# jennalandy/bayesNMF

Measured on AMD Instinct MI355X. Metric: Gibbs iters/sec at K=96, G=10k, N=20; per-chain scaling at 1/2/4/8 GPUs, higher is better.
Workload: dtype f64; 1 GPU; Poisson-Gamma fixed rank N=20, K=96 x G=10000 synthetic counts, one chain per GPU, stats mode, record_sample into a 1000-deep device ring (on) and a metrics row every iteration; chains=1, seed=1, sum_M=40006177, record_window=1000

## Files before the change

bayesnmf_amd/csrc/api.hip:

```cpp
#include <hip/hip_runtime.h>
#include <hip/hip_ext.h>
#include <chrono>
#include <climits>
#include <cmath>
#include <cstdarg>
#include <cstdio>
#include <cstdlib>
#include <cstring>
#include <cerrno>
#include <algorithm>
#include <map>
#include <atomic>
#include <condition_variable>
#include <mutex>
#include <string>
#include <thread>
#include <vector>
#include <fcntl.h>
#include <sys/file.h>
#include <sys/stat.h>
#include <unistd.h>
#include "kernels.h"
#include "zalloc_reg.h"
#include "zalloc_sort.h"
// ... 47 lines not shown
  DevPool& P = g_pool[dev];
  {
    std::lock_guard<std::mutex> lk(P.m);
    auto it = P.free_blocks.find(bytes);
    if (it != P.free_blocks.end()) { *out = it->second; P.free_blocks.erase(it); P.cached -= bytes; P.live[*out] = bytes; return hipSuccess; }
  }
  hipError_t e = hipMalloc(out, bytes);
  if (e != hipSuccess) { (void)hipGetLastError(); pool_drop(dev); e = hipMalloc(out, bytes); }
  if (e == hipSuccess) { std::lock_guard<std::mutex> lk(P.m); P.live[*out] = bytes; }
  return e;
}
template <class T> static hipError_t dmalloc(T** out, size_t bytes) { return dmalloc_raw((void**)out, bytes); }
static hipError_t dfree(void* p) {
  if (!p) return hipSuccess;
  int dev = -1;
  if (hipGetDevice(&dev) != hipSuccess || dev < 0 || dev >= 64) return hipFree(p);
  DevPool& P = g_pool[dev];
  {
    std::lock_guard<std::mutex> lk(P.m);
    auto it = P.live.find(p);
    if (it != P.live.end()) {
      const size_t bytes = it->second;
      P.live.erase(it);
      if (P.cached + bytes <= pool_cap()) { P.free_blocks.insert({bytes, p}); P.cached += bytes; return hipSuccess; }
    }
  }
  return hipFree(p);
}


#include "zplan.h"

struct Arr { double* d = nullptr; size_t n = 0; int stride = 1; bool set = false; std::vector<int> redraw; double* ring = nullptr;
             bool slab = false; };

struct Pipe {
  bool side_valid = false, side_main = false, flags_valid = false, side_ev_stale = false;
  int gate_f0 = 1;
  uint32_t z_gate_next = 0, z_gated_for = 0;
  bool red_pending = false, red_issued = false, red_on_side2 = false; uint32_t red_t = 0; int red_row = 0;
  uint32_t ct_pending = 0, mh_etail_pending = 0;
  bool mh_prep_valid = false, mh_pipe_valid = false;
  int z_expanded_iter = 0;
  void invalidate_prepared() { side_valid = false; side_main = false; mh_prep_valid = false; mh_pipe_valid = false; }
};

enum class ZKind { none , general , reg , tile, step, sort };

struct ZTile : ZTilePlan { double* dMhat = nullptr; };
struct ZSort {
  bool pk = false, shared = false;
  ZSGeom g{}; int nblk = 0, w = 0; size_t lds = 0;
  int it16 = 0, qmax = ZS_QMAX;
  int nempty = 0;
  uint32_t* dItems = nullptr; ZSBlock* dBlocks = nullptr; int* dCols = nullptr; int32_t* dM = nullptr; unsigned long long* dProf = nullptr;
  double* dMh = nullptr;
  uint32_t *dRec = nullptr, *dRecRing = nullptr; size_t recwords = 0; bool eager = false;
  int x_cols = 0; size_t x_lds = 0;
};
struct ZStep {
  ZPGeom g{}; int ns = 0 , gbp = 0; size_t lds = 0; bool it16 = false;
  uint32_t* dItems = nullptr; ZPWg* dWgs = nullptr; ZPBatch* dBatches = nullptr; ZPStep* dSteps = nullptr; int* dCols = nullptr;
};
struct Rank : RankPlan { double *dCol = nullptr, *dMhat = nullptr; uint32_t* dSync = nullptr; void* dDbg = nullptr; };
struct Mh : MhPlan {
  bool side_tail = true;
  bool side_main = true;
  bool no_reg = false;
  bool e_k128 = false;
  int e_gw = 0;
  double *dMhat = nullptr, *dAccPn = nullptr, *dAccEpart = nullptr, *dEt = nullptr; int* dNzE = nullptr;
  int32_t* dMt = nullptr; double* dMtf = nullptr;
};

struct Scratch { unsigned char* p = nullptr; size_t bytes = 0; };

struct bnmf_handle {
  bnmf_config cfg{};
  int device = 0;
  hipStream_t stream = nullptr;
  hipStream_t side = nullptr;
  hipStream_t side2 = nullptr;
  hipEvent_t ev_draw = nullptr, ev_side = nullptr, ev_sideP = nullptr, ev_p = nullptr, ev_z = nullptr, ev_red = nullptr, ev_rank = nullptr;
  std::vector<void*> owned;
  int gate_forced = -1;
  int draw_bw = 0;
  double* dScal = nullptr;
  unsigned* dDrawOwn = nullptr; unsigned draw_seq = 0;
  int dbg_draw_no_p = 0;
  int dbg_main_delay_us = 0;
  int dbg_allside_delay_us = 0;
  int dbg_side_delay_us = 0;
  double* E_alt = nullptr;
  const void* z_attr_kernel = nullptr;
  Pipe pipe;
  int iter = 0;
  bool inited = false;
  Dev dev{};
  Arr arr[BNMF_ID_MAX];
  int32_t *dM = nullptr, *dZsumK = nullptr, *dZsumG = nullptr, *dZ = nullptr;
  double* dMf = nullptr;
  int* dR = nullptr; int* dRedraw = nullptr;
  std::vector<int32_t> fixedP;
  int n_fixed = 0; int* dFixedP = nullptr;
  double *dEsum = nullptr, *dPsum = nullptr, *dlpPn = nullptr, *dlpE = nullptr, *dcol = nullptr;
  double* hMetrics = nullptr;
// ... 189 lines not shown
  if (int rc = check_args("bnmf_create", cfg, M, out)) return rc;
  return create_handle(cfg, M, nullptr, out);
}

int bnmf_create_f64(const bnmf_config* cfg, const double* M, bnmf_handle** out) {
  if (int rc = check_args("bnmf_create_f64", cfg, M, out)) return rc;
  const size_t K = cfg->K, G = cfg->G;
  if (cfg->likelihood == BNMF_NORMAL) {
    for (size_t g = 0; g < G; ++g)
      for (size_t k = 0; k < K; ++k)
        if (!std::isfinite(M[k + K * g])) return fail(BNMF_EINVAL, "bnmf_create_f64: M[%zu, %zu] = %g is not finite", k, g, M[k + K * g]);
    return create_handle(cfg, nullptr, M, out);
  }
  if (cfg->likelihood != BNMF_POISSON) return fail(BNMF_EMODEL, "likelihood must be one of normal, poisson");
  std::vector<int32_t> mi(K * G);
  for (size_t g = 0; g < G; ++g)
    for (size_t k = 0; k < K; ++k) {
      const double v = M[k + K * g];
      if (!(v >= 0.0 && v <= 2147483647.0 && v == std::floor(v)))
        return fail(BNMF_EINVAL, "bnmf_create_f64: non-integer count M[%zu, %zu] = %g (likelihood = poisson takes whole numbers in [0, 2^31 - 1])", k, g, v);
      mi[k + K * g] = (int32_t)v;
    }
  return bnmf_create(cfg, mi.data(), out);
}

static int build_zsort(bnmf_handle* h, const int32_t* M, bool reg_ok, const Switches& sw) {
  const bnmf_config& c = h->cfg;
  const size_t K = c.K, G = c.G, N = c.N;
  ZSort& z = h->zs;
  ZSortPlan p;
  if (int rc = plan_zsort(M, K, G, N, c.save_Z != 0, h->maxM, reg_ok, h->n_cu, sw, p)) return rc;
  if (!p.ok) return 0;
  if (p.it16) HIPCHK(hupload(h, &z.dItems, p.items16.data(), p.items16.size() * sizeof(uint16_t), (p.items16.size() * sizeof(uint16_t) + 3) & ~(size_t)3));
  else HIPCHK(hupload(h, &z.dItems, p.items.data(), p.items.size() * sizeof(uint32_t)));
  z.it16 = p.it16 ? 1 : 0; z.qmax = p.qmax;
  HIPCHK(hupload(h, &z.dBlocks, p.blocks.data(), p.blocks.size() * sizeof(ZSBlock)));
  HIPCHK(hupload(h, &z.dCols, p.cols.data(), p.cols.size() * sizeof(int)));
  HIPCHK(hupload(h, &z.dM, p.Mblk.data(), p.Mblk.size() * sizeof(int32_t)));
  HIPCHK(hzeroed(h, &z.dMh, 3 * K * G * sizeof(double)));
  if (c.save_Z) {
    const size_t hw = (N + 1) / 2;
    z.recwords = p.items.size() * hw;
    HIPCHK(hmalloc(h, &z.dRec, z.recwords * sizeof(uint32_t)));
    z.eager = sw.z_eager;
    const size_t lds_max = 160 * 1024;
    z.x_cols = std::max(1, std::min(p.GBc, zexpand_cols((int)K, (int)N, lds_max)));
    z.x_lds = ((size_t)z.x_cols * N * ((K + 1) / 2) * 4 + 15) & ~(size_t)15;
    if (z.x_lds > lds_max) return fail(BNMF_EINVAL, "bnmf_create: K = %zu, N = %zu: a column of Z does not fit the LDS of k_zexpand", K, N);
    HIPCHK(hipFuncSetAttribute((const void*)k_zexpand, hipFuncAttributeMaxDynamicSharedMemorySize, 160 * 1024));
  }
  z.g = ZSGeom{p.KP, p.GBc, p.nb};
  z.shared = p.shared;
  z.nblk = p.nblk; z.w = p.W; z.pk = p.pk; z.nempty = p.nempty;
  z.lds = (zsort_shared_bytes((int)K, (int)N, p.KP, p.GBc, p.pk) + (size_t)p.W * zsort_wave_bytes(p.nblk, (int)N) + 15) & ~(size_t)15;
  h->zkind = ZKind::sort;
#ifdef ZSPROF
  HIPCHK(hzeroed(h, &z.dProf, (8 + 3 * 16 * 8) * sizeof(unsigned long long)));
#endif
  return 0;
}

static int build_zstep(bnmf_handle* h, const int32_t* M, const Switches& sw) {
  const bnmf_config& c = h->cfg;
  ZStep& z = h->zp;
  ZStepPlan p;
  if (int rc = plan_zstep(M, c.K, c.G, c.N, c.save_Z != 0, h->n_cu, sw, p)) return rc;
  if (!p.ok) return 0;
  z.it16 = p.it16;
  if (p.it16) HIPCHK(hupload(h, &z.dItems, p.items16.data(), p.items16.size() * sizeof(uint16_t), (p.items16.size() * sizeof(uint16_t) + 3) & ~(size_t)3));
  else HIPCHK(hupload(h, &z.dItems, p.items.data(), p.items.size() * sizeof(uint32_t)));
  HIPCHK(hupload(h, &z.dWgs, p.wgs.data(), p.wgs.size() * sizeof(ZPWg)));
  HIPCHK(hupload(h, &z.dBatches, p.batches.data(), p.batches.size() * sizeof(ZPBatch)));
  HIPCHK(hupload(h, &z.dSteps, p.steps.data(), p.steps.size() * sizeof(ZPStep)));
  HIPCHK(hupload(h, &z.dCols, p.cols.data(), p.cols.size() * sizeof(int)));
  z.g = ZPGeom{p.nch, p.nwg, nullptr};
#ifdef ZPPROF
  HIPCHK(hzeroed(h, &z.g.prof, 8 * sizeof(unsigned long long)));
#endif
  z.ns = p.W; z.gbp = p.GBP;
  z.lds = (zstep_shared_bytes((int)c.N, p.GBP) + p.W * zstep_wave_bytes(p.L) + 15) & ~(size_t)15;
  h->zkind = ZKind::step;
  return 0;
}

static std::mutex g_stream_mtx;
static std::vector<hipStream_t> g_stream_pool[64];
static int take_stream(int device, hipStream_t* out, int kind = 0) {
  (void)kind;
  if (device < 0 || device >= 64) return fail(BNMF_EINVAL, "device ordinal %d out of range", device);
  {
    std::lock_guard<std::mutex> lock(g_stream_mtx);
    auto& v = g_stream_pool[device];
    if (!v.empty()) { *out = v.back(); v.pop_back(); return 0; }
  }
  HIPCHK(hipStreamCreateWithFlags(out, hipStreamNonBlocking));
  return 0;
}
static void give_stream(int device, hipStream_t st, int kind = 0) {
  (void)kind;
  if (!st) return;
  if (device < 0 || device >= 64) { hipStreamDestroy(st); return; }
  std::lock_guard<std::mutex> lock(g_stream_mtx);
  g_stream_pool[device].push_back(st);
}
struct CachedBuf { void* p; size_t bytes; };
static std::mutex g_ring_mtx;
// ... 1017 lines not shown
```

bayesnmf_amd/csrc/sweep.h:

```cpp
#include <cassert>

static int need_hyper(bnmf_handle* h, std::initializer_list<int> ids) {
  for (int id : ids) if (!h->arr[id].d) return fail(BNMF_EUNSET, "hyper-prior array id %d was not set (fill_hyperprior_params, R/setup.R:15-88)", id);
  return 0;
}
static int ensure_metrics(bnmf_handle* h, size_t rows) {
  if (rows <= h->metrics_rows) return 0;
  HIPCHK(hipStreamSynchronize(h->stream));
  HIPCHK(hipHostFree(h->hMetrics));
  h->hMetrics = nullptr; h->dMetrics = nullptr;
  h->metrics_rows = rows;
  HIPCHK(hipHostMalloc((void**)&h->hMetrics, rows * BNMF_NMETRIC * sizeof(double), hipHostMallocMapped));
  HIPCHK(hipHostGetDevicePointer((void**)&h->dMetrics, h->hMetrics, 0));
  HIPCHK(hfree(h, h->dRaw));
  HIPCHK(hmalloc(h, &h->dRaw, rows * 8 * sizeof(double)));
  refresh_dev(h);
  return 0;
}
static void set_slot(const bnmf_handle* h, Dev& d, uint32_t t) {
  const size_t sl = t % 3u, G = h->cfg.G, N = h->cfg.N;
  d.colsse = h->dcol + sl * 3 * G; d.colll = d.colsse + G; d.colkl = d.colsse + 2 * G;
  d.lpE_part = h->dlpE + sl * (size_t)h->nblkE;
  d.lpPn = h->dlpPn + sl * N;
}
// ... 204 lines not shown
}
template <bool SZ, int ZT_, bool LEAN_>
static int launch_ztile(bnmf_handle* h, uint32_t t) {
  auto kern = k_zalloc_tile<SZ, ZT_, LEAN_>;
  if (int rc = raise_lds_limit(h, (const void*)kern)) return rc;
  const ZArgs za = zargs(h);
  hipLaunchKernelGGL(kern, dim3(h->zt.grid), dim3(ZT_), h->zt.lds, h->stream, za, h->zt.dMhat, t, h->zt.g);
  hipLaunchKernelGGL(k_colmetrics<256>, dim3((h->cfg.G + 3) / 4), dim3(256), 0, h->stream, za, (const double*)h->zt.dMhat);
  if (h->zt.g.dbg) {
    unsigned long long v[8];
    hipStreamSynchronize(h->stream);
    hipMemcpy(v, h->zt.g.dbg, sizeof v, hipMemcpyDeviceToHost);
    hipMemset(h->zt.g.dbg, 0, sizeof v);
    if (v[0]) fprintf(stderr, "[ztile t=%u] waves %llu grid %d w %d lds %zu  per wave: phase1 %.1f  phase2 %.1f  flush %.1f  columns %.1f  kernel %.1f (s_memtime ticks)\n",
                      t, v[0], h->zt.grid, h->zt.w, h->zt.lds, (double)v[1] / v[0], (double)v[2] / v[0], (double)v[3] / v[0], (double)v[4] / v[0], (double)v[5] / v[0]);
  }
  return 0;
}
template <bool SZ, int ZT_>
static int launch_zalloc_t(bnmf_handle* h, uint32_t t) {
  if (h->zkind == ZKind::tile) return (h->zt.lean && ZT_ == 1024) ? launch_ztile<SZ, ZT_, (ZT_ == 1024)>(h, t) : launch_ztile<SZ, ZT_, false>(h, t);
  if (h->zkind == ZKind::general) return launch_z(h, t, k_zalloc<SZ, ZT_>, h->dev, ZT_);
#ifdef BNMF_DIAG
  if (h->z_ablate) return launch_zreg_t<SZ, ZT_, true>(h, t);
#endif
  return launch_zreg_t<SZ, ZT_, false>(h, t);
}
static int zs_prio() { static const int v = getenv("BNMF_ZSPRIO") ? atoi(getenv("BNMF_ZSPRIO")) : 1; return v; }
static uint32_t* zs_rec_at(const bnmf_handle* h, uint32_t t) {
  if (!h->zs.dRec) return nullptr;
  return h->zs.dRecRing ? h->zs.dRecRing + (size_t)((t - 1) % (uint32_t)h->wcap) * h->zs.recwords : h->zs.dRec;
}
static void launch_zexpand(bnmf_handle* h, uint32_t t) {
  const ZSArgs sa{zargs(h), h->zs.dItems, h->zs.dBlocks, h->zs.dCols, h->zs.dM, h->zs.it16, h->zs.qmax, zs_rec_at(h, t), nullptr, 0, 0, h->zs.dProf};
  hipLaunchKernelGGL(k_zexpand, dim3(h->zs.g.nblocks), dim3(ZX_T), h->zs.x_lds, h->stream, sa, h->zs.x_cols);
  h->pipe.z_expanded_iter = (int)t;
}
static int ensure_Z(bnmf_handle* h) {
  if (h->zkind != ZKind::sort || !h->zs.dRec || !h->cfg.save_Z || h->iter < 1 || h->pipe.z_expanded_iter == h->iter) return 0;
  HIPCHK(hipSetDevice(h->device));
  launch_zexpand(h, (uint32_t)h->iter);
  HIPCHK(hipGetLastError());
  HIPCHK(hipStreamSynchronize(h->stream));
  return 0;
}
template <int ZT_>
static int launch_zsort_t(bnmf_handle* h, uint32_t t) {
  const ZSArgs sa{zargs(h), h->zs.dItems, h->zs.dBlocks, h->zs.dCols, h->zs.dM, h->zs.it16, h->zs.qmax, zs_rec_at(h, t), h->zs.dMh + (size_t)(t % 3u) * h->cfg.K * h->cfg.G, zs_prio(), h->zs.shared ? 1 : 0, h->zs.dProf};
  auto go = [&](auto kern) -> int {
    if (int rc = raise_lds_limit(h, (const void*)kern)) return rc;
    hipLaunchKernelGGL(kern, dim3(h->zs.g.nblocks), dim3(ZT_), h->zs.lds, h->stream, sa, t, h->zs.g);
    return 0;
  };
#ifdef BNMF_FASTBUILD
  if (h->zs.nblk != 4) return fail(BNMF_EMODEL, "BNMF_FASTBUILD: only N = 16..20");
  return h->zs.pk ? go(k_zalloc_sort<ZT_, 4, true>) : go(k_zalloc_sort<ZT_, 4, false>);
#else
  if (h->zs.pk) switch (h->zs.nblk) {
    case 1: return go(k_zalloc_sort<ZT_, 1, true>);
    case 2: return go(k_zalloc_sort<ZT_, 2, true>);
    case 3: return go(k_zalloc_sort<ZT_, 3, true>);
    case 4: return go(k_zalloc_sort<ZT_, 4, true>);
    default: return go(k_zalloc_sort<ZT_, 5, true>);
  }
  switch (h->zs.nblk) {
    case 1: return go(k_zalloc_sort<ZT_, 1, false>);
    case 2: return go(k_zalloc_sort<ZT_, 2, false>);
    case 3: return go(k_zalloc_sort<ZT_, 3, false>);
    case 4: return go(k_zalloc_sort<ZT_, 4, false>);
    default: return go(k_zalloc_sort<ZT_, 5, false>);
  }
#endif
}
static int launch_zsort(bnmf_handle* h, uint32_t t) {
#ifdef BNMF_FASTBUILD
  if (h->zs.w == 14) return launch_zsort_t<896>(h, t);
  if (h->zs.w != 12) return fail(BNMF_EMODEL, "BNMF_FASTBUILD: only 12 or 14 waves");
  return launch_zsort_t<768>(h, t);
#else
  switch (h->zs.w) {
    case 16: return launch_zsort_t<1024>(h, t);
    case 14: return launch_zsort_t<896>(h, t);
    case 12: return launch_zsort_t<768>(h, t);
    case 8: return launch_zsort_t<512>(h, t);
    case 6: return launch_zsort_t<384>(h, t);
    default: return launch_zsort_t<256>(h, t);
  }
#endif
}
static int launch_zstep(bnmf_handle* h, uint32_t t) {
  const ZPArgs pa{zargs(h), h->zp.dItems, h->zp.it16 ? 1 : 0, h->zp.dWgs, h->zp.dBatches, h->zp.dSteps, h->zp.dCols};
  auto go = [&](auto kern) -> int {
    if (int rc = raise_lds_limit(h, (const void*)kern)) return rc;
    hipLaunchKernelGGL(kern, dim3(h->zp.g.nwg), dim3(h->zp.ns * 64), h->zp.lds, h->stream, pa, t, h->zp.g);
    return 0;
  };
  return h->zp.gbp == 40 ? go(k_zalloc_step<4, 40, 8>) : go(k_zalloc_step<4, 32, 8>);
}
static int launch_zalloc(bnmf_handle* h, uint32_t t) {
  int w = 0;
  switch (h->zkind) {
    case ZKind::none: return fail(BNMF_ESTATE, "launch_zalloc: the handle allocates no counts");
    case ZKind::sort:
      if (int rc = launch_zsort(h, t)) return rc;
      if (h->cfg.save_Z && h->zs.eager) launch_zexpand(h, t);
      return 0;
// ... 466 lines not shown
```

bayesnmf_amd/csrc/zalloc_sort.h:

```cpp
#pragma once

namespace bnmf {

constexpr int ZS_QMAX = 32;
constexpr int ZS_QMAX16 = 64;
constexpr int ZS_NMAX = 25;

struct ZSBlock { int item0, ntask, col0, ncols; };
struct ZSGeom { int KP, GBc, nblocks; };
struct ZSArgs {
  ZArgs a;
  const uint32_t* items;
  const ZSBlock* blocks;
  const int* cols;
  const int32_t* Mblk;
  int it16, qmax;
  uint32_t* rec;
  double* mh;
  int prio;
  int shared;
  unsigned long long* prof;
};
#ifdef ZSPROF
#define ZSTIC(i) const uint64_t zstic_##i = __builtin_amdgcn_s_memtime()
#define ZSTOC(i) zsprof[i] += __builtin_amdgcn_s_memtime() - zstic_##i
#define ZSSTAMP(j) do { if (s.prof && zs_sel >= 0 && lane == 0) s.prof[8 + (zs_sel * 16 + wave) * 8 + (j)] = __builtin_amdgcn_s_memrealtime(); } while (0)
#else
#define ZSTIC(i)
#define ZSTOC(i)
#define ZSSTAMP(j)
#endif
#define BNMF_HD __host__ __device__ inline
BNMF_HD int zsort_zrows(int N, bool pk) { return pk ? (N + 1) / 2 : N; }
BNMF_HD size_t zsort_shared_bytes(int K, int N, int KP, int GBc, bool pk) {
  size_t w = (size_t)zsort_zrows(N, pk) * (KP + GBc) + GBc + 4;
  w = (w + 3) & ~(size_t)3;
  return (w * 4 + ((size_t)K * N + (size_t)N * GBc) * 8 + 15) & ~(size_t)15;
}
BNMF_HD size_t zsort_wave_bytes(int NBLK, int N) { return (size_t)NBLK * 64 * 16 + (size_t)(2 * ((N + 1) / 2)) * 64 * 4; }

template <int ZT, int NBLK , bool PK>
__global__ __launch_bounds__(ZT) __attribute__((amdgpu_waves_per_eu(4))) void k_zalloc_sort(ZSArgs s, uint32_t t, ZSGeom zg) {
  constexpr int NPV = NBLK - 1;
  constexpr int NC = 5 * NBLK;
  constexpr int NMIN = NBLK == 1 ? 1 : 5 * (NBLK - 1) + 1;
  extern __shared__ __attribute__((aligned(16))) unsigned char smem[];
  const ZArgs& d = s.a;
  const int tid = threadIdx.x, lane = tid & 63, wave = tid >> 6;
  const int K = d.K, N = d.N, KP = zg.KP, GBc = zg.GBc;
  const int HW = (N + 1) >> 1;
  const int ZR = PK ? HW : N;
  const ZSBlock bk = s.blocks[blockIdx.x];
  uint32_t* zG = (uint32_t*)smem;
  uint32_t* zK = zG + (size_t)ZR * KP;
  int* colid = (int*)(zK + (size_t)ZR * GBc);
  uint32_t* ticket = (uint32_t*)(colid + GBc);
  const size_t w32 = (((size_t)ZR * (KP + GBc) + GBc + 4) + 3) & ~(size_t)3;
  const int32_t* Mb = s.Mblk + (size_t)K * bk.col0;
  double* Pl = (double*)(smem + w32 * 4);
  double* ae = Pl + (size_t)K * N;
  unsigned char* wbase = smem + zsort_shared_bytes(K, N, KP, GBc, PK) + (size_t)wave * zsort_wave_bytes(NBLK, N);
  u4* tblk = (u4*)wbase;
  uint32_t* hist = (uint32_t*)(tblk + NBLK * 64);
#ifdef ZSPROF
  uint64_t zsprof[8] = {0, 0, 0, 0, 0, 0, 0, 1};
#endif
#ifdef ZSPROF
  int zs_ntask = 0;
  const int zs_sel = blockIdx.x == 0 ? 0 : blockIdx.x == 128 ? 1 : blockIdx.x == gridDim.x - 1 ? 2 : -1;
#endif
  ZSSTAMP(0);
  ZSTIC(6);
  ZSTIC(0);
  for (int i = lane; i < 2 * HW * 64; i += 64) hist[i] = 0;
  {
    constexpr int UA = 2, UP = 4;
    const int nP = K * N, nA = N * bk.ncols;
    const int nchunk = max(max((nA + UA * ZT - 1) / (UA * ZT), (nP + UP * ZT - 1) / (UP * ZT)), 1);
    for (int ch = 0; ch < nchunk; ++ch) {
      int gcol[UA], an_i[UA], ax[UA];
      double an[UA], pv[UP], ev[UA];
#pragma unroll
      for (int u = 0; u < UA; ++u) {
        const int i = (ch * UA + u) * ZT + tid;
        const bool ok = i < nA;
        const int gl = ok ? i / N : 0, n = ok ? i - gl * N : 0;
        ax[u] = ok ? n * GBc + gl : -1; an_i[u] = n;
        gcol[u] = s.cols[bk.col0 + gl];
        an[u] = d.A[n];
      }
#pragma unroll
      for (int u = 0; u < UP; ++u) { const int i = (ch * UP + u) * ZT + tid; pv[u] = i < nP ? d.P[i] : 0.0; }
#pragma unroll
      for (int u = 0; u < UA; ++u) ev[u] = d.E[an_i[u] + (size_t)N * gcol[u]];
#pragma unroll
      for (int u = 0; u < UP; ++u) { const int i = (ch * UP + u) * ZT + tid; if (i < nP) Pl[i] = pv[u]; }
#pragma unroll
      for (int u = 0; u < UA; ++u) if (ax[u] >= 0) ae[ax[u]] = an[u] * ev[u];
    }
    for (int i = tid; i < bk.ncols; i += ZT) colid[i] = s.cols[bk.col0 + i];
    for (int i = tid; i < ZR * KP; i += ZT) zG[i] = 0;
    for (int i = tid; i < ZR * GBc; i += ZT) zK[i] = 0;
    if (tid == 0) *ticket = 0;
  }
  ZSSTAMP(1);
  __syncthreads();
  ZSTOC(0);
  ZSSTAMP(2);
  if (s.prio) __builtin_amdgcn_s_setprio(2);
  const int nthr = N - 1;
  const int ntot = bk.ntask;
  const uint32_t hlb = lds_off(hist + lane);
  auto next_task = [&]() -> int {
    int tk = 0;
    if (lane == 0) tk = (int)__hip_atomic_fetch_add(ticket, 1u, __ATOMIC_RELAXED, __HIP_MEMORY_SCOPE_WORKGROUP);
    return __builtin_amdgcn_readlane(tk, 0);
  };
  for (int task = next_task(); task < ntot; task = next_task()) {
    {
    ZSTIC(1);
    uint32_t it;
    if (s.it16) {
      const uint32_t r = ((const uint16_t*)s.items)[(size_t)bk.item0 + (size_t)task * 64 + lane];
      it = r == 0xFFFFu ? 0xFFFFFFFFu : ((r & 127u) | (((r >> 7) & 63u) << 10) | ((r >> 13) << 16));
    } else it = s.items[(size_t)bk.item0 + (size_t)task * 64 + lane];
    const bool valid = it != 0xFFFFFFFFu;
    const int k = valid ? (int)(it & 1023u) : 0, gl = valid ? (int)((it >> 10) & 63u) : 0;
    const int q0 = valid ? (int)(it >> 16) * s.qmax : 0;
    const int m = Mb[k + (size_t)K * gl];
    const int g = colid[gl];
    int nq = 0, npad = 0;
    bool any = false;
    uint32_t pv[NPV > 0 ? NPV : 1];
    {
      const double* Pk = Pl + k;
      const double* ag = ae + gl;
      double cs[NC];
      double c = 0.0;
#pragma unroll
      for (int n = 0; n < NC; ++n) { if (n < NMIN || n < N) c = c + Pk[(size_t)K * n] * ag[(size_t)n * GBc]; cs[n] = c; }
      if (valid && c > 0.0 && m > 0) {
        const int qt = (m + 3) >> 2;
        nq = min(s.qmax, qt - q0);
        npad = (q0 + nq == qt) ? ((4 - (m & 3)) & 3) : 0;
      }
      if (valid && q0 == 0) s.mh[(size_t)k + (size_t)K * (size_t)g] = c;
      any = __builtin_amdgcn_ballot_w64(nq > 0) != 0;
      if (any) {
      const double scale = 4294967296.0 / c;
#pragma unroll
      for (int j = 0; j < NBLK; ++j) {
        uint32_t tv[5];
#pragma unroll
        for (int i = 0; i < 5; ++i) {
          const int n = 5 * j + i;
          tv[i] = 0xFFFFFFFFu;
          if (n < NC - 1 && (n < NMIN - 1 || n < nthr)) tv[i] = cvt_u32_sat(cs[n] * scale);
        }
        tblk[j * 64 + lane] = u4{tv[0], tv[1], tv[2], tv[3]};
        if (j < NPV) pv[j] = tv[4];
      }
      }
    }
    const uint32_t celem = (uint32_t)k + (uint32_t)K * (uint32_t)g;
    auto quad = [&](int qidx, uint32_t inc0, uint32_t inc1, uint32_t inc2, uint32_t inc3) {
      const u32x4 w = philox4x32_7((uint32_t)qidx, celem, t, BNMF_V_Z, d.k0, d.k1);
      const uint32_t u0 = min(w.x, 0xFFFFFFFEu), u1 = min(w.y, 0xFFFFFFFEu), u2 = min(w.z, 0xFFFFFFFEu), u3 = min(w.w, 0xFFFFFFFEu);
      uint32_t j0 = 0, j1 = 0, j2 = 0, j3 = 0;
#pragma unroll
      for (int p = 0; p < NPV; ++p) cmp_acc4(pv[p], u0, u1, u2, u3, j0, j1, j2, j3);
      const u4 k0 = tblk[j0 * 64 + lane], k1 = tblk[j1 * 64 + lane], k2 = tblk[j2 * 64 + lane], k3 = tblk[j3 * 64 + lane];
      const uint32_t b0 = 5 * j0 + (k0.x <= u0) + (k0.y <= u0) + (k0.z <= u0) + (k0.w <= u0);
      const uint32_t b1 = 5 * j1 + (k1.x <= u1) + (k1.y <= u1) + (k1.z <= u1) + (k1.w <= u1);
      const uint32_t b2 = 5 * j2 + (k2.x <= u2) + (k2.y <= u2) + (k2.z <= u2) + (k2.w <= u2);
      const uint32_t b3 = 5 * j3 + (k3.x <= u3) + (k3.y <= u3) + (k3.z <= u3) + (k3.w <= u3);
      lds_add(mad24(b0, 256, hlb), inc0);
      lds_add(mad24(b1, 256, hlb), inc1);
      lds_add(mad24(b2, 256, hlb), inc2);
      lds_add(mad24(b3, 256, hlb), inc3);
    };
    wave_lds_fence();
    ZSTOC(1);
#ifdef ZSPROF
    if (zs_ntask == 0) ZSSTAMP(6);
#endif
    ZSTIC(2);
    if (any) for (int i = 0; __builtin_amdgcn_ballot_w64(i < nq - 1) != 0; ++i)
      if (i < nq - 1) quad(q0 + i, 1u, 1u, 1u, 1u);
    if (nq > 0) quad(q0 + nq - 1, 1u, npad > 2 ? 0u : 1u, npad > 1 ? 0u : 1u, npad > 0 ? 0u : 1u);
    wave_lds_fence();
    ZSTOC(2);
#ifdef ZSPROF
    if (zs_ntask == 0) ZSSTAMP(7);
    ++zs_ntask;
#endif
    ZSTIC(3);
    if (s.rec) {
      uint32_t* rt = s.rec + ((size_t)(bk.item0 >> 6) + (size_t)task) * (size_t)HW * 64 + lane;
      for (int w = 0; w < HW; ++w) rt[(size_t)w * 64] = hist[(2 * w) * 64 + lane] | (hist[(2 * w + 1) * 64 + lane] << 16);
    }
    if (nq > 0) {
      const uint32_t zgb = lds_off(zG) + ((uint32_t)k << 2), zkb = lds_off(zK) + ((uint32_t)gl << 2);
      for (int w = 0; w < HW; ++w) {
        const uint32_t v0 = hist[(2 * w) * 64 + lane], v1 = hist[(2 * w + 1) * 64 + lane];
        const uint32_t v = v0 | (v1 << 16);
        if (v) {
          hist[(2 * w) * 64 + lane] = 0; hist[(2 * w + 1) * 64 + lane] = 0;
          if (PK) {
            lds_add(zgb + (uint32_t)w * (uint32_t)KP * 4u, v); lds_add(zkb + (uint32_t)w * (uint32_t)GBc * 4u, v);
          } else {
            const uint32_t lo = v & 0xFFFFu, hi = v >> 16;
            if (lo) { lds_add(zgb + (uint32_t)(2 * w) * (uint32_t)KP * 4u, lo); lds_add(zkb + (uint32_t)(2 * w) * (uint32_t)GBc * 4u, lo); }
            if (hi) { lds_add(zgb + (uint32_t)(2 * w + 1) * (uint32_t)KP * 4u, hi); lds_add(zkb + (uint32_t)(2 * w + 1) * (uint32_t)GBc * 4u, hi); }
          }
        }
      }
    }
    wave_lds_fence();
    ZSTOC(3);
    }
  }
  ZSSTAMP(3);
  ZSTIC(5);
  __syncthreads();
  ZSTOC(5);
  ZSSTAMP(4);
  {
  ZSTIC(0);
  for (int i = tid; i < N * bk.ncols; i += ZT) {
    const int gl = i / N, n = i - gl * N;
    const uint32_t v = PK ? (zK[(size_t)(n >> 1) * GBc + gl] >> ((n & 1) << 4)) & 0xFFFFu : zK[(size_t)n * GBc + gl];
    if (s.shared) { if (v) atomicAdd(&d.ZsumK[n + (size_t)N * colid[gl]], (int32_t)v); }
    else d.ZsumK[n + (size_t)N * colid[gl]] = (int32_t)v;
  }
  for (int i = tid; i < K * N; i += ZT) {
    const int kk = i % K, n = i / K;
    const uint32_t v = PK ? (zG[(size_t)(n >> 1) * KP + kk] >> ((n & 1) << 4)) & 0xFFFFu : zG[(size_t)n * KP + kk];
    if (v) atomicAdd(&d.ZsumG[kk + (size_t)K * n], (int32_t)v);
  }
  ZSTOC(0);
  }
  ZSTOC(6);
  ZSSTAMP(5);
#ifdef ZSPROF
  if (s.prof && lane == 0) for (int i = 0; i < 8; ++i) atomicAdd(&s.prof[i], (unsigned long long)zsprof[i]);
#endif
  if (d.gate0 && blockIdx.x == 0 && tid == 0) {
    unsigned spins = 0;
    while (__hip_atomic_load(d.gate0, __ATOMIC_RELAXED, __HIP_MEMORY_SCOPE_AGENT) < d.gate_epoch ||
           __hip_atomic_load(d.gate1, __ATOMIC_RELAXED, __HIP_MEMORY_SCOPE_AGENT) < d.gate_epoch) {
      __builtin_amdgcn_s_sleep(2);
      if (++spins > (1u << 24)) { __hip_atomic_store(d.gate_err, 2, __ATOMIC_RELAXED, __HIP_MEMORY_SCOPE_AGENT); break; }
    }
  }
}

constexpr int ZX_T = 1024;
BNMF_HD int zexpand_cols(int K, int N, size_t lds_bytes) { return (int)(lds_bytes / ((size_t)N * (size_t)((K + 1) / 2) * 4)); }
__global__ __launch_bounds__(ZX_T) void k_zexpand(ZSArgs s, int cols_per_pass) {
  extern __shared__ __attribute__((aligned(16))) unsigned char smem[];
  uint32_t* slab = (uint32_t*)smem;
  const ZArgs& d = s.a;
  const int tid = threadIdx.x, K = d.K, N = d.N, KH = (K + 1) >> 1, HW = (N + 1) >> 1;
  const ZSBlock bk = s.blocks[blockIdx.x];
  const int nslots = bk.ntask * 64;
  for (int c0 = 0; c0 < bk.ncols; c0 += cols_per_pass) {
    const int nc = min(cols_per_pass, bk.ncols - c0);
    for (int i = tid; i < nc * N * KH; i += ZX_T) slab[i] = 0u;
    __syncthreads();
    for (int i = tid; i < nslots; i += ZX_T) {
      uint32_t it;
      if (s.it16) { const uint32_t r = ((const uint16_t*)s.items)[(size_t)bk.item0 + i]; it = r == 0xFFFFu ? 0xFFFFFFFFu : ((r & 127u) | (((r >> 7) & 63u) << 10)); }
      else it = s.items[(size_t)bk.item0 + i];
      if (it == 0xFFFFFFFFu) continue;
      const int k = (int)(it & 1023u), gl = (int)((it >> 10) & 63u) - c0;
      if (gl < 0 || gl >= nc) continue;
      const uint32_t* rt = s.rec + ((size_t)((bk.item0 + i) >> 6)) * (size_t)HW * 64 + (i & 63);
      uint32_t* sc = slab + (size_t)gl * N * KH + (k >> 1);
      const int sh = (k & 1) << 4;
      for (int w = 0; w < HW; ++w) {
        const uint32_t v = rt[(size_t)w * 64];
        if (v & 0xFFFFu) atomicAdd(sc + (size_t)(2 * w) * KH, (v & 0xFFFFu) << sh);
        if (v >> 16) atomicAdd(sc + (size_t)(2 * w + 1) * KH, (v >> 16) << sh);
      }
    }
// ... 23 lines not shown
```

bayesnmf_amd/csrc/zplan.h:

```cpp

static const int ENV_UNSET = INT_MIN;
static bool env_set(const char* name) { return getenv(name) != nullptr; }
static int env_int(const char* name, int unset = ENV_UNSET, int lo = INT_MIN, int hi = INT_MAX) {
  const char* e = getenv(name);
  return e ? std::max(lo, std::min(hi, atoi(e))) : unset;
}
static bool env_flag(const char* name, bool unset) { const char* e = getenv(name); return e ? atoi(e) != 0 : unset; }
static double env_real(const char* name, double unset) { const char* e = getenv(name); return e ? atof(e) : unset; }
struct Switches {
  bool devlock = true;
  int gate = -1, serial = -1;
  bool mh_side_main = true, mh_side_tail = true;
  bool draw_no_p = false;
  int main_delay_us = 0, allside_delay_us = 0, side_delay_us = 0;
  bool rank_dbg = false, zt_dbg = false;
  bool z_eager = false;
  int ablate = 0;
  bool rank_half = true; long rank_grid = 0;
  bool mhe_k128 = false, mh_pipe = true; int mhe_gw = 0;
  bool z_reg = true, z_chunk = false, z_tile = true, z_nolean = false;
  int zw = ENV_UNSET, z_grid = ENV_UNSET;
  bool zsort = true, zs_spread = true, zs_it16 = true, zs_pk = true;
  int zs_lds_kb = ENV_UNSET, zs_w = ENV_UNSET, zs_qmax = 0;
  bool zstep = true, zp_it16 = true; int zp_gb = 0;
  static Switches from_env() {
    Switches s;
    s.devlock = env_flag("BNMF_DEVLOCK", true);
    s.gate = env_set("BNMF_GATE") ? (int)env_flag("BNMF_GATE", false) : -1;
    s.serial = env_set("BNMF_SERIAL") ? (int)env_flag("BNMF_SERIAL", false) : -1;
    s.mh_side_main = env_flag("BNMF_MHSIDE", true); s.mh_side_tail = env_flag("BNMF_MHSIDETAIL", true);
    s.draw_no_p = env_flag("BNMF_DEBUG_DRAW_NO_P", false);
    s.main_delay_us = env_int("BNMF_DEBUG_MAIN_DELAY_US", 0, 0, 20000);
    s.allside_delay_us = env_int("BNMF_DEBUG_ALLSIDE_DELAY_US", 0, 0, 20000);
    s.side_delay_us = env_int("BNMF_DEBUG_SIDE_DELAY_US", 0, 0, 20000);
    s.rank_dbg = env_set("BNMF_RANKDBG"); s.zt_dbg = env_set("BNMF_ZTDBG");
    s.z_eager = env_flag("BNMF_ZEAGER", false);
#ifdef BNMF_DIAG
    s.ablate = env_int("BNMF_ABLATE", 0);
#endif
    s.rank_half = env_flag("BNMF_RANKHALF", true);
    if (const char* e = getenv("BNMF_RANKGRID")) s.rank_grid = atol(e);
    s.mhe_k128 = env_flag("BNMF_MHE_K128", false); s.mh_pipe = env_flag("BNMF_MHPIPE", true);
    { const int v = env_int("BNMF_MHE_GW", 0); s.mhe_gw = v == 32 ? 32 : v == 16 ? 16 : 0; }
    s.z_reg = env_flag("BNMF_ZREG", true); s.z_chunk = env_flag("BNMF_ZCHUNK", false);
    s.z_tile = env_flag("BNMF_ZTILE", true); s.z_nolean = env_set("BNMF_ZNOLEAN");
    s.zw = env_int("BNMF_ZW"); s.z_grid = env_int("BNMF_ZGRID");
    s.zsort = env_flag("BNMF_ZSORT", true); s.zs_spread = env_flag("BNMF_ZSSPREAD", true);
    s.zs_it16 = env_flag("BNMF_ZSIT16", true); s.zs_pk = env_flag("BNMF_ZSPK", true);
    s.zs_lds_kb = env_int("BNMF_ZSLDS"); s.zs_w = env_int("BNMF_ZSW"); s.zs_qmax = env_int("BNMF_ZSQMAX", 0);
    s.zstep = env_flag("BNMF_ZSTEP", true); s.zp_it16 = env_flag("BNMF_ZPIT16", true); s.zp_gb = env_int("BNMF_ZPGB", 0);
    return s;
  }
};

struct RankPlan { bool reg = false, half = false; int grid = 0; };
static RankPlan plan_rank(size_t K, size_t G, int n_cu, int occ_reg, int occ_gen, const Switches& sw) {
  RankPlan p;
  const long NB = ((long)G + RK_MAXC - 1) / RK_MAXC;
  const long wg_needed = (NB + RK_CW - 1) / RK_CW;
  auto cap = [&](int occ) { return (long)std::min(1, occ >= 6 ? occ - 1 : occ) * n_cu; };
  const long cap_reg = cap(occ_reg), cap_gen = cap(occ_gen);
  p.reg = K <= 96 && wg_needed <= cap_reg;
  const long wg_half = (NB + RK_CWH / 2 - 1) / (RK_CWH / 2);
  p.half = p.reg && wg_half <= (long)n_cu && NB <= 1536 && sw.rank_half;
  const long cap_used = p.reg ? cap_reg : cap_gen;
  p.grid = p.half ? (int)wg_half : (int)std::min<long>(wg_needed, cap_used);
  if (!p.half && sw.rank_grid >= wg_needed && sw.rank_grid <= cap_used) p.grid = (int)sw.rank_grid;
  return p;
}

struct MhPlan {
  int S = 1;
  size_t e_lds = 0;
  bool e16 = false;
  bool e_raise = false, e16_raise = false;
  bool pipe = false;
};
static int plan_mh(size_t K, size_t G, size_t N, bool poisson_mh_fixed_rank, bool side_main, bool side_tail, const Switches& sw, MhPlan& p) {
  p = MhPlan();
  p.S = (int)((G + MH_SEG - 1) / MH_SEG);
  p.e_lds = 4 * (2 * N + 3 * K) * sizeof(double);
  if (p.e_lds > 160 * 1024) return fail(BNMF_EINVAL, "bnmf_create: K = %zu too large for the column kernel of the MH / Normal models (LDS)", K);
  p.e_raise = p.e_lds > 64 * 1024;
  const size_t lds16_max = (4 * (size_t)4 * N * (1 + PRE_W) + 2 * N) * sizeof(double);
  p.e16 = K <= (size_t)MHE16_KMAX && lds16_max <= 160 * 1024;
  p.e16_raise = p.e16 && lds16_max > 64 * 1024;
  p.pipe = p.e16 && poisson_mh_fixed_rank && side_main && side_tail && N <= RT && sw.mh_pipe;
  return 0;
}

struct ZWavePlan {
  bool reg = false;
  ZGeom g{};
  int w = 8, per_cu = 0, grid = 0;
  size_t lds = 0;
};
static int plan_zwave(size_t K, size_t G, size_t N, bool save_Z, int n_cu, const Switches& sw, ZWavePlan& p) {
  p = ZWavePlan();
  ZGeom& zg = p.g;
  zg.KP = (K % 32 == 0) ? (int)K + 1 : (int)(K | 1);
  zg.HW = (int)((N + 3) / 4);
// ... 410 lines not shown
```

Measured before the change: 12230 Gibbs iterations/s (aggregate over chains).

## Add compile-time specialized zalloc_sort kernel for K=96, N=20 geometries

Adds a template trait that fixes K, N, KP, GBc, it16, qmax, prio, shared and rec as compile-time constants, so the Z-allocation sort kernel can constant-fold its index math. When every lane in a wave has quads, the fixed path processes two Philox draws per iteration up to the wave-minimum count, giving more instruction-level parallelism. It also flushes the packed histogram into zG/zK with an unrolled, register-staged loop. The specialization is chosen at setup only for two exact geometries and falls back to the generic kernel otherwise. This adds more template instantiations, and the specialized kernel may use more registers.

Result: faster. 12460 Gibbs iterations/s (aggregate over chains) (median of 6 runs) (+1.9%).

```diff
diff --git a/bayesnmf_amd/csrc/api.hip b/bayesnmf_amd/csrc/api.hip
--- a/bayesnmf_amd/csrc/api.hip
+++ b/bayesnmf_amd/csrc/api.hip
@@ -123,6 +123,7 @@
   bool pk = false, shared = false;
   ZSGeom g{}; int nblk = 0, w = 0; size_t lds = 0;
   int it16 = 0, qmax = ZS_QMAX;
+  int fixed = 0;
   int nempty = 0;
   uint32_t* dItems = nullptr; ZSBlock* dBlocks = nullptr; int* dCols = nullptr; int32_t* dM = nullptr; unsigned long long* dProf = nullptr;
   double* dMh = nullptr;
@@ -418,6 +419,7 @@
   z.g = ZSGeom{p.KP, p.GBc, p.nb};
   z.shared = p.shared;
   z.nblk = p.nblk; z.w = p.W; z.pk = p.pk; z.nempty = p.nempty;
+  z.fixed = sw.zs_fixed ? zsort_fixed_form((int)K, (int)N, p.KP, p.GBc, z.it16, p.qmax, p.W, p.nblk, p.pk, p.shared, c.save_Z != 0) : 0;
   z.lds = (zsort_shared_bytes((int)K, (int)N, p.KP, p.GBc, p.pk) + (size_t)p.W * zsort_wave_bytes(p.nblk, (int)N) + 15) & ~(size_t)15;
   h->zkind = ZKind::sort;
 #ifdef ZSPROF
diff --git a/bayesnmf_amd/csrc/sweep.h b/bayesnmf_amd/csrc/sweep.h
--- a/bayesnmf_amd/csrc/sweep.h
+++ b/bayesnmf_amd/csrc/sweep.h
@@ -280,6 +280,13 @@
     hipLaunchKernelGGL(kern, dim3(h->zs.g.nblocks), dim3(ZT_), h->zs.lds, h->stream, sa, t, h->zs.g);
     return 0;
   };
+  if constexpr (ZT_ == ZSFIX_ZT) {
+    if (h->zs.fixed && sa.prio != 0 && !sa.rec && !sa.shared) switch (h->zs.fixed) {
+      case 1: return go(k_zalloc_sort<ZSFIX_ZT, ZSFIX_NBLK, true, ZSFix10k>);
+      case 2: return go(k_zalloc_sort<ZSFIX_ZT, ZSFIX_NBLK, true, ZSFix2k>);
+      default: break;
+    }
+  }
 #ifdef BNMF_FASTBUILD
   if (h->zs.nblk != 4) return fail(BNMF_EMODEL, "BNMF_FASTBUILD: only N = 16..20");
   return h->zs.pk ? go(k_zalloc_sort<ZT_, 4, true>) : go(k_zalloc_sort<ZT_, 4, false>);
diff --git a/bayesnmf_amd/csrc/zalloc_sort.h b/bayesnmf_amd/csrc/zalloc_sort.h
--- a/bayesnmf_amd/csrc/zalloc_sort.h
+++ b/bayesnmf_amd/csrc/zalloc_sort.h
@@ -39,15 +39,48 @@
 }
 BNMF_HD size_t zsort_wave_bytes(int NBLK, int N) { return (size_t)NBLK * 64 * 16 + (size_t)(2 * ((N + 1) / 2)) * 64 * 4; }
 
-template <int ZT, int NBLK , bool PK>
+struct ZSDyn {
+  static constexpr bool fixed = false, prio = false, shared = false, rec = false;
+  static constexpr int K = 0, N = 0, KP = 0, GBc = 0, IT16 = 0, QMAX = 0;
+};
+template <int K_, int N_, int KP_, int GBc_, int IT16_, int QMAX_, bool PRIO_ = true, bool SHARED_ = false, bool REC_ = false>
+struct ZSFixed {
+  static constexpr bool fixed = true, prio = PRIO_, shared = SHARED_, rec = REC_;
+  static constexpr int K = K_, N = N_, KP = KP_, GBc = GBc_, IT16 = IT16_, QMAX = QMAX_;
+};
+constexpr int ZSFIX_ZT = 896, ZSFIX_NBLK = 4;
+using ZSFix10k = ZSFixed<96, 20, 97, 40, 1, 64>;
+using ZSFix2k = ZSFixed<96, 20, 97, 8, 0, 16>;
+template <class FX>
+inline bool zsort_fixed_is(int K, int N, int KP, int GBc, int it16, int qmax) {
+  return K == FX::K && N == FX::N && KP == FX::KP && GBc == FX::GBc && (it16 != 0) == (FX::IT16 != 0) && qmax == FX::QMAX;
+}
+inline int zsort_fixed_form(int K, int N, int KP, int GBc, int it16, int qmax, int W, int nblk, bool pk, bool shared, bool rec) {
+  if (!pk || shared || rec || W * 64 != ZSFIX_ZT || nblk != ZSFIX_NBLK) return 0;
+  return zsort_fixed_is<ZSFix10k>(K, N, KP, GBc, it16, qmax) ? 1 : zsort_fixed_is<ZSFix2k>(K, N, KP, GBc, it16, qmax) ? 2 : 0;
+}
+BNMF_DEV int wave_min_i32(int v) {
+  v = min(v, __builtin_amdgcn_update_dpp(v, v, 0xB1, 0xf, 0xf, false));
+  v = min(v, __builtin_amdgcn_update_dpp(v, v, 0x4E, 0xf, 0xf, false));
+  v = min(v, __builtin_amdgcn_update_dpp(v, v, 0x141, 0xf, 0xf, false));
+  v = min(v, __builtin_amdgcn_update_dpp(v, v, 0x140, 0xf, 0xf, false));
+  return min(min(__builtin_amdgcn_readlane(v, 0), __builtin_amdgcn_readlane(v, 16)), min(__builtin_amdgcn_readlane(v, 32), __builtin_amdgcn_readlane(v, 48)));
+}
+
+template <int ZT, int NBLK , bool PK, class FX = ZSDyn >
 __global__ __launch_bounds__(ZT) __attribute__((amdgpu_waves_per_eu(4))) void k_zalloc_sort(ZSArgs s, uint32_t t, ZSGeom zg) {
+  constexpr bool FIX = FX::fixed;
+  static_assert(!FIX || (NBLK == (FX::N + 4) / 5 && FX::N >= 1 && FX::N < ZS_NMAX && FX::K >= 1 && FX::GBc >= 1 && FX::GBc <= 64 && FX::QMAX >= 1), "ZSFixed: geometry");
   constexpr int NPV = NBLK - 1;
   constexpr int NC = 5 * NBLK;
   constexpr int NMIN = NBLK == 1 ? 1 : 5 * (NBLK - 1) + 1;
   extern __shared__ __attribute__((aligned(16))) unsigned char smem[];
   const ZArgs& d = s.a;
   const int tid = threadIdx.x, lane = tid & 63, wave = tid >> 6;
-  const int K = d.K, N = d.N, KP = zg.KP, GBc = zg.GBc;
+  const int K = FIX ? FX::K : d.K, N = FIX ? FX::N : d.N, KP = FIX ? FX::KP : zg.KP, GBc = FIX ? FX::GBc : zg.GBc;
+  const int qmax = FIX ? FX::QMAX : s.qmax;
+  const bool it16 = FIX ? FX::IT16 != 0 : s.it16 != 0, prio = FIX ? FX::prio : s.prio != 0, shared = FIX ? FX::shared : s.shared != 0;
+  const bool rec = FIX ? FX::rec : s.rec != nullptr;
   const int HW = (N + 1) >> 1;
   const int ZR = PK ? HW : N;
   const ZSBlock bk = s.blocks[blockIdx.x];
@@ -107,7 +140,7 @@
   __syncthreads();
   ZSTOC(0);
   ZSSTAMP(2);
-  if (s.prio) __builtin_amdgcn_s_setprio(2);
+  if (prio) __builtin_amdgcn_s_setprio(2);
   const int nthr = N - 1;
   const int ntot = bk.ntask;
   const uint32_t hlb = lds_off(hist + lane);
@@ -120,13 +153,13 @@
     {
     ZSTIC(1);
     uint32_t it;
-    if (s.it16) {
+    if (it16) {
       const uint32_t r = ((const uint16_t*)s.items)[(size_t)bk.item0 + (size_t)task * 64 + lane];
       it = r == 0xFFFFu ? 0xFFFFFFFFu : ((r & 127u) | (((r >> 7) & 63u) << 10) | ((r >> 13) << 16));
     } else it = s.items[(size_t)bk.item0 + (size_t)task * 64 + lane];
     const bool valid = it != 0xFFFFFFFFu;
     const int k = valid ? (int)(it & 1023u) : 0, gl = valid ? (int)((it >> 10) & 63u) : 0;
-    const int q0 = valid ? (int)(it >> 16) * s.qmax : 0;
+    const int q0 = valid ? (int)(it >> 16) * qmax : 0;
     const int m = Mb[k + (size_t)K * gl];
     const int g = colid[gl];
     int nq = 0, npad = 0;
@@ -141,7 +174,7 @@
       for (int n = 0; n < NC; ++n) { if (n < NMIN || n < N) c = c + Pk[(size_t)K * n] * ag[(size_t)n * GBc]; cs[n] = c; }
       if (valid && c > 0.0 && m > 0) {
         const int qt = (m + 3) >> 2;
-        nq = min(s.qmax, qt - q0);
+        nq = min(qmax, qt - q0);
         npad = (q0 + nq == qt) ? ((4 - (m & 3)) & 3) : 0;
       }
       if (valid && q0 == 0) s.mh[(size_t)k + (size_t)K * (size_t)g] = c;
@@ -163,7 +196,7 @@
       }
     }
     const uint32_t celem = (uint32_t)k + (uint32_t)K * (uint32_t)g;
-    auto quad = [&](int qidx, uint32_t inc0, uint32_t inc1, uint32_t inc2, uint32_t inc3) {
+    auto find = [&](int qidx, uint32_t& a0, uint32_t& a1, uint32_t& a2, uint32_t& a3) {
       const u32x4 w = philox4x32_7((uint32_t)qidx, celem, t, BNMF_V_Z, d.k0, d.k1);
       const uint32_t u0 = min(w.x, 0xFFFFFFFEu), u1 = min(w.y, 0xFFFFFFFEu), u2 = min(w.z, 0xFFFFFFFEu), u3 = min(w.w, 0xFFFFFFFEu);
       uint32_t j0 = 0, j1 = 0, j2 = 0, j3 = 0;
@@ -174,10 +207,15 @@
       const uint32_t b1 = 5 * j1 + (k1.x <= u1) + (k1.y <= u1) + (k1.z <= u1) + (k1.w <= u1);
       const uint32_t b2 = 5 * j2 + (k2.x <= u2) + (k2.y <= u2) + (k2.z <= u2) + (k2.w <= u2);
       const uint32_t b3 = 5 * j3 + (k3.x <= u3) + (k3.y <= u3) + (k3.z <= u3) + (k3.w <= u3);
-      lds_add(mad24(b0, 256, hlb), inc0);
-      lds_add(mad24(b1, 256, hlb), inc1);
-      lds_add(mad24(b2, 256, hlb), inc2);
-      lds_add(mad24(b3, 256, hlb), inc3);
+      a0 = mad24(b0, 256, hlb); a1 = mad24(b1, 256, hlb); a2 = mad24(b2, 256, hlb); a3 = mad24(b3, 256, hlb);
+    };
+    auto quad = [&](int qidx, uint32_t inc0, uint32_t inc1, uint32_t inc2, uint32_t inc3) {
+      uint32_t a0, a1, a2, a3;
+      find(qidx, a0, a1, a2, a3);
+      lds_add(a0, inc0);
+      lds_add(a1, inc1);
+      lds_add(a2, inc2);
+      lds_add(a3, inc3);
     };
     wave_lds_fence();
     ZSTOC(1);
@@ -185,7 +223,21 @@
     if (zs_ntask == 0) ZSSTAMP(6);
 #endif
     ZSTIC(2);
-    if (any) for (int i = 0; __builtin_amdgcn_ballot_w64(i < nq - 1) != 0; ++i)
+    int i = 0;
+    if constexpr (FIX) {
+      if (__builtin_amdgcn_ballot_w64(nq > 0) == ~0ull) {
+        const int nfull = wave_min_i32(nq - 1);
+        for (; i + 1 < nfull; i += 2) {
+          uint32_t a0, a1, a2, a3, c0, c1, c2, c3;
+          find(q0 + i, a0, a1, a2, a3);
+          find(q0 + i + 1, c0, c1, c2, c3);
+          lds_add(a0, 1u); lds_add(a1, 1u); lds_add(a2, 1u); lds_add(a3, 1u);
+          lds_add(c0, 1u); lds_add(c1, 1u); lds_add(c2, 1u); lds_add(c3, 1u);
+        }
+        if (i < nfull) { quad(q0 + i, 1u, 1u, 1u, 1u); ++i; }
+      }
+    }
+    if (any) for (; __builtin_amdgcn_ballot_w64(i < nq - 1) != 0; ++i)
       if (i < nq - 1) quad(q0 + i, 1u, 1u, 1u, 1u);
     if (nq > 0) quad(q0 + nq - 1, 1u, npad > 2 ? 0u : 1u, npad > 1 ? 0u : 1u, npad > 0 ? 0u : 1u);
     wave_lds_fence();
@@ -195,11 +247,24 @@
     ++zs_ntask;
 #endif
     ZSTIC(3);
-    if (s.rec) {
+    if (rec) {
       uint32_t* rt = s.rec + ((size_t)(bk.item0 >> 6) + (size_t)task) * (size_t)HW * 64 + lane;
       for (int w = 0; w < HW; ++w) rt[(size_t)w * 64] = hist[(2 * w) * 64 + lane] | (hist[(2 * w + 1) * 64 + lane] << 16);
     }
-    if (nq > 0) {
+    if constexpr (FIX && PK) {
+      if (nq > 0) {
+        constexpr int HWC = (FX::N + 1) >> 1;
+        const uint32_t zgb = lds_off(zG) + ((uint32_t)k << 2), zkb = lds_off(zK) + ((uint32_t)gl << 2);
+        uint32_t v[HWC];
+#pragma unroll
+        for (int w = 0; w < HWC; ++w) v[w] = hist[(2 * w) * 64 + lane] | (hist[(2 * w + 1) * 64 + lane] << 16);
+#pragma unroll
+        for (int w = 0; w < HWC; ++w) if (v[w]) {
+          hist[(2 * w) * 64 + lane] = 0; hist[(2 * w + 1) * 64 + lane] = 0;
+          lds_add(zgb + (uint32_t)w * (uint32_t)FX::KP * 4u, v[w]); lds_add(zkb + (uint32_t)w * (uint32_t)FX::GBc * 4u, v[w]);
+        }
+      }
+    } else if (nq > 0) {
       const uint32_t zgb = lds_off(zG) + ((uint32_t)k << 2), zkb = lds_off(zK) + ((uint32_t)gl << 2);
       for (int w = 0; w < HW; ++w) {
         const uint32_t v0 = hist[(2 * w) * 64 + lane], v1 = hist[(2 * w + 1) * 64 + lane];
@@ -230,7 +295,7 @@
   for (int i = tid; i < N * bk.ncols; i += ZT) {
     const int gl = i / N, n = i - gl * N;
     const uint32_t v = PK ? (zK[(size_t)(n >> 1) * GBc + gl] >> ((n & 1) << 4)) & 0xFFFFu : zK[(size_t)n * GBc + gl];
-    if (s.shared) { if (v) atomicAdd(&d.ZsumK[n + (size_t)N * colid[gl]], (int32_t)v); }
+    if (shared) { if (v) atomicAdd(&d.ZsumK[n + (size_t)N * colid[gl]], (int32_t)v); }
     else d.ZsumK[n + (size_t)N * colid[gl]] = (int32_t)v;
   }
   for (int i = tid; i < K * N; i += ZT) {
diff --git a/bayesnmf_amd/csrc/zplan.h b/bayesnmf_amd/csrc/zplan.h
--- a/bayesnmf_amd/csrc/zplan.h
+++ b/bayesnmf_amd/csrc/zplan.h
@@ -21,6 +21,7 @@
   bool z_reg = true, z_chunk = false, z_tile = true, z_nolean = false;
   int zw = ENV_UNSET, z_grid = ENV_UNSET;
   bool zsort = true, zs_spread = true, zs_it16 = true, zs_pk = true;
+  bool zs_fixed = true;
   int zs_lds_kb = ENV_UNSET, zs_w = ENV_UNSET, zs_qmax = 0;
   bool zstep = true, zp_it16 = true; int zp_gb = 0;
   static Switches from_env() {
@@ -46,7 +47,7 @@
     s.z_tile = env_flag("BNMF_ZTILE", true); s.z_nolean = env_set("BNMF_ZNOLEAN");
     s.zw = env_int("BNMF_ZW"); s.z_grid = env_int("BNMF_ZGRID");
     s.zsort = env_flag("BNMF_ZSORT", true); s.zs_spread = env_flag("BNMF_ZSSPREAD", true);
-    s.zs_it16 = env_flag("BNMF_ZSIT16", true); s.zs_pk = env_flag("BNMF_ZSPK", true);
+    s.zs_it16 = env_flag("BNMF_ZSIT16", true); s.zs_pk = env_flag("BNMF_ZSPK", true); s.zs_fixed = env_flag("BNMF_ZSFIXED", true);
     s.zs_lds_kb = env_int("BNMF_ZSLDS"); s.zs_w = env_int("BNMF_ZSW"); s.zs_qmax = env_int("BNMF_ZSQMAX", 0);
     s.zstep = env_flag("BNMF_ZSTEP", true); s.zp_it16 = env_flag("BNMF_ZPIT16", true); s.zp_gb = env_int("BNMF_ZPGB", 0);
     return s;
```
